# SmallEndian/antidote

Hardware: AMD Instinct MI355X
Metric: CRDT ops materialized/sec (whole node) + % HBM peak (higher is better)
Workload: dtype u64; 1 GPU; c3: antidote_crdt_set_aw, 1048576 keys x 1024 ops per GPU, D=8, 64-element universe; keys_per_gpu=1048576, ops_per_gpu=1073741824, n_dc=8, partitions=64, parallelism=partition-sharded x1, key_placement=rank r holds the keys with am_key_partition(key, 64) % N == r, step=GST min all-reduce (RCCL) + materialize all keys, base=fresh, zone_index=none

## Files before the change

### antidote_amd/csrc/am_group_split.h

```cpp
#pragma once

namespace amk_grp {

constexpr uint32_t IWB = 32;
__device__ __forceinline__ uint32_t wave_min_u32_v(uint32_t v) {
#define S_(C) v = min(v, dpp32<C>(v));
  AMK_ROW_STEPS(S_)
#undef S_
  v = min(v, (uint32_t)__shfl_xor((int)v, 16, WAVE));
  return min(v, (uint32_t)__shfl_xor((int)v, 32, WAVE));
}
struct ISlot {
  uint64_t off0, K, idb, key;
  uint32_t r, nops;
};
constexpr int SEGT = 4;
constexpr uint32_t SEGOPS = SEGT * 256;
template <int DMAX, bool LAG>
struct ISred {
  uint32_t mx[DMAX][WAVE];
};
template <int DMAX>
struct ISred<DMAX, true> {
  union {
    uint32_t mx[DMAX][WAVE];
    uint16_t list[SEGOPS];
  };
  uint32_t stage[SEGOPS / 32];
};
template <int DMAX, bool LAG>
struct ISmem : ISred<DMAX, LAG> {
  ISlot slot[IWB];
  uint64_t ct[DMAX][IWB];
  uint64_t mex[IWB];
  uint32_t count[IWB], pres[IWB];
  uint32_t flags[IWB];
};

template <int DMAX, int OPL, bool RANGE, class Ent>
__device__ __forceinline__ uint32_t incl_tile(const Ent &x, const PkRead<DMAX> &pk, uint64_t g, uint64_t off0,
                                              uint64_t off1, uint32_t (&mx)[DMAX], uint32_t &esc, uint32_t &cand) {
  uint32_t ib = 0;
#pragma unroll
  for (int k = 0; k < OPL; ++k) {
    const bool e = x.esc(k) == AM_PK_ESC;
    const bool inr = !RANGE || (g + k >= off0 && g + k < off1);
    bool in = inr && !e;
#pragma unroll
    for (int d = 0; d < DMAX; ++d) in = in && x(k, d) <= pk.thr[d];
    esc |= (uint32_t)(inr && e) << k;
    cand |= (uint32_t)(inr && !e) << k;
    if (in) {
#pragma unroll
      for (int d = 0; d < DMAX; ++d) mx[d] = max(mx[d], x(k, d));
    }
    ib |= (uint32_t)in << k;
  }
  return ib;
}

template <int DMAX>
__device__ __forceinline__ uint32_t mx_reduce(const uint32_t (*smx)[WAVE], uint32_t lane) {
  uint32_t m = 0;
  {
    const uint32_t d = lane >> 3, c = lane & 7u;
    if (d < (uint32_t)DMAX) {
      const u32x4 a0 = *(const u32x4 *)&smx[d][8 * c], a1 = *(const u32x4 *)&smx[d][8 * c + 4];
      m = max(max(max(a0.x, a0.y), max(a0.z, a0.w)), max(max(a1.x, a1.y), max(a1.z, a1.w)));
    }
    m = max(m, dpp32<0xB1>(m));
    m = max(m, dpp32<0x4E>(m));
    m = max(m, dpp32<0x141>(m));
  }
  uint32_t ql = lane;
  asm volatile("" : "+v"(ql));
  return (uint32_t)__builtin_amdgcn_ds_bpermute((int)((ql & 7u) << 5), (int)m);
}

#ifndef AM_INCL_WAVES
#define AM_INCL_WAVES(D) 4
#endif
#ifndef AM_INCL_LAG_WAVES
#define AM_INCL_LAG_WAVES(D) 5
#endif
template <int DMAX, int TYPE, bool EXACT, bool LAG>
__global__ void __launch_bounds__(BLOCK, LAG ? AM_INCL_LAG_WAVES(DMAX) : AM_INCL_WAVES(DMAX)) k_grp_incl(am_log_arg LA, am_read_batch B, am_read_result R, am_sel S,
                                                       am_retry next, am_retry routed, uint32_t short_opl,
                                                       uint32_t *ibm, uint64_t *escr) {
  const am_op_log L = LA.log();
  constexpr int OPL = 4;
  constexpr uint64_t TILE = (uint64_t)WAVE * OPL;
  constexpr uint32_t LPW = 32 / OPL;
  __shared__ ISmem<DMAX, LAG> smem[NW];
  ISmem<DMAX, LAG> &sm = smem[threadIdx.x >> 6];
  ISlot *sl = sm.slot;
  const uint32_t lane = threadIdx.x & (WAVE - 1);
  const uint32_t nd = EXACT ? (uint32_t)DMAX : L.n_dc;
  const uint64_t stride = L.snap_stride ? L.snap_stride : L.n_ops;
  const uint32_t sel0 = S.idx ? uniform_u32(S.range[0]) : 0u;
  const uint64_t nsel = S.idx ? (uint64_t)(uniform_u32(S.range[1]) - sel0) : B.n_reads;
  const uint64_t W = (uint64_t)gridDim.x * NW;
  const uint64_t gw = (uint64_t)blockIdx.x * NW + uniform_u32(threadIdx.x >> 6);
  const uint64_t n = B.n_reads;
  ReadU<DMAX> u;
  read_inputs<DMAX, false, true>(L, nd, B, 0, u);

  for (uint64_t b0 = gw * IWB; b0 < nsel; b0 += (uint64_t)IWB * W) {
    uint32_t sl_ = lane, sopl = short_opl;
    asm volatile("" : "+v"(sl_));
    asm volatile("" : "+s"(sopl));
    const uint64_t ii = b0 + sl_;
    bool elig = false, hand = false, route = false;
    uint64_t rr = 0;
    if (sl_ < IWB && ii < nsel) {
      GMeta mm;
      read_meta(L, B, S.idx ? (uint64_t)S.idx[sel0 + ii] : ii, TYPE, mm);
      rr = mm.r;
      if (mm.st != AM_OK) {
        R.status[mm.r] = mm.st, R.flags[mm.r] = 0;
      } else if (!wave_takes(L, B, mm, sopl)) {
        hand = true;
      } else if (LAG && routed.list && L.key_lag[mm.key * nd] == AM_LAG_ROUTED) {
        route = true;
      } else {
        elig = true;
        ISlot &w = sl[sl_];
        w.off0 = mm.off0, w.K = L.key_tbase[mm.key], w.idb = L.key_id_base ? L.key_id_base[mm.key] : 1;
        w.key = mm.key;
        w.r = (uint32_t)mm.r, w.nops = (uint32_t)(mm.off1 - mm.off0);
      }
    }
    const uint64_t hm = __ballot(hand);
    if (hm) {
      uint32_t base = 0;
      if (sl_ == 0) base = atomicAdd(next.count, (uint32_t)__popcll(hm));
      base = uniform_u32(base);
      if (hand) next.list[base + (uint32_t)__popcll(hm & ((1ull << sl_) - 1ull))] = (uint32_t)rr;
    }
    if (LAG) retry_append(routed, route, (uint32_t)rr, sl_);
    const uint64_t emask = __ballot(elig);
    uint32_t escmask = 0;
    uint64_t *const escw = escr + (gw * IWB) * WAVE;
    wave_sync();

    for (uint64_t em = emask; em; em &= em - 1) {
      const uint32_t j = (uint32_t)__builtin_ctzll(em);
      const uint64_t off0 = uniform_u64(sl[j].off0), off1 = off0 + uniform_u32(sl[j].nops);
      PkRead<DMAX> pk;
      pk_setup(u, nd, uniform_u64(sl[j].K), pk);
      uint32_t lb[DMAX];
      if (LAG) {
        const uint64_t key = uniform_u64(sl[j].key);
#pragma unroll
        for (int d = 0; d < DMAX; ++d) lb[d] = uniform_u32(d < (int)nd ? (uint32_t)L.key_lag[key * nd + d] : 0u);
      }
      uint32_t cnt = 0, minex = 0xFFFFFFFFu, anyc = 0, anyesc = 0;
      uint32_t mxr = 0;
      uint64_t escm = 0;
      const uint64_t t0 = off0 & ~31ull;
      if constexpr (LAG) {
        static_assert(OPL == 4 && TILE == 256 && SEGOPS == SEGT * TILE, "list entries: tile, lane, op of four");
        int64_t cinf = AM_IW_NOBOUND;
        int32_t lbm = INT32_MAX;
#pragma unroll
        for (int d = 0; d < DMAX; ++d)
          if (d < (int)nd) cinf = am_iw_fold(cinf, pk.thr[d], lb[d]), lbm = min(lbm, (int32_t)lb[d]);
        am_inclwin iw;
        am_iw_init(&iw, cinf, pk.never);
        const uint32_t cin_lim = am_iw_lim(iw.cin), out_lim = am_iw_lim(iw.hi);
        uint32_t in_lim = am_iw_in_lim(&iw);
        const uint32_t lo = (uint32_t)(off0 - t0), nops = (uint32_t)(off1 - off0);
        uint16_t *const list = sm.list;
        uint32_t *const stage = sm.stage;
        const uint32_t nt = (uint32_t)((off1 - 1 - t0) / TILE) + 1u;
        for (uint32_t sg = (nt + SEGT - 1) / SEGT; sg-- > 0;) {
          const uint64_t sb = t0 + (uint64_t)sg * SEGOPS;
          const uint32_t sr = sg * SEGOPS;
          uint32_t c[SEGT][OPL];
#pragma unroll
          for (int k = 0; k < SEGT; ++k) {
            const uint64_t g = sb + (uint64_t)k * TILE + (uint64_t)lane * OPL;
#pragma unroll
            for (int i = 0; i < OPL; ++i) c[k][i] = 0;
            if (g < off1) ld_n32<OPL>(L.lag_ct + g, c[k]);
          }
          if (in_lim < cin_lim) {
            uint32_t sure = 0;
#pragma unroll
            for (int k = 0; k < SEGT; ++k)
#pragma unroll
              for (int i = 0; i < OPL; ++i) {
                const uint32_t q = sr + (uint32_t)k * (uint32_t)TILE + lane * OPL + (uint32_t)i;
                if (q - lo < nops && c[k][i] < cin_lim) sure = max(sure, c[k][i] + 1u);
              }
            const uint32_t m = uniform_u32(wave_max_u32_v(sure));
            if (m) am_iw_raise(&iw, am_iw_cmax_sure(m - 1u)), in_lim = am_iw_in_lim(&iw);
          }
          uint32_t nl = 0;
          auto classify = [&](const int k, const uint32_t (&ck)[OPL]) {
            const uint64_t t = sb + (uint64_t)k * TILE;
            if (t >= off1) return;
            const uint32_t q = sr + (uint32_t)k * (uint32_t)TILE + lane * OPL;
            uint32_t *const sw = stage + k * (int)(TILE / 32) + lane / LPW;
            const bool whole = t >= off0 && t + TILE <= off1;
            if (whole) {
              const uint32_t ch = max(max(ck[0], ck[1]), max(ck[2], ck[3]));
              const uint32_t cl = min(min(ck[0], ck[1]), min(ck[2], ck[3]));
              const bool in = !__ballot(ch >= in_lim);
              if (in || !__ballot(cl < out_lim || ch == AM_PK_ESC)) {
                if (in) cnt += OPL;
                else minex = min(minex, q);
                anyc |= (1u << OPL) - 1u;
                if (lane % LPW == 0) *sw = in ? ~0u : 0u;
                return;
              }
            }
            uint32_t esc = 0, cand = 0, ib = 0, win = 0;
#pragma unroll
            for (int i = 0; i < OPL; ++i) {
              const bool inr = whole || q + (uint32_t)i - lo < nops;
              const int cl = am_iw_class32(ck[i], in_lim, out_lim);
              esc |= (uint32_t)(inr && cl == AM_IW_ESCAPED) << i;
              cand |= (uint32_t)(inr && cl != AM_IW_ESCAPED) << i;
              ib |= (uint32_t)(inr && cl == AM_IW_IN) << i;
              win |= (uint32_t)(inr && cl == AM_IW_WINDOW) << i;
            }
            cnt += (uint32_t)__popc(ib);
            anyc |= cand;
            anyesc |= esc;
            const uint32_t ti = q / (uint32_t)TILE;
            if (esc) escm |= ti < 64 / OPL ? (uint64_t)esc << (OPL * ti) : ~0ull;
            const uint32_t ex = cand & ~ib & ~win;
            if (ex) minex = min(minex, q + (uint32_t)__builtin_ctz(ex));
            uint32_t word = ib << (OPL * (lane % LPW));
#pragma unroll
            for (uint32_t xo = 1; xo < LPW; xo <<= 1) word |= (uint32_t)__shfl_xor((int)word, (int)xo);
            if (lane % LPW == 0) *sw = word;
            if (__ballot(win != 0)) {
              const uint32_t pc = (uint32_t)__popc(win);
              const uint32_t inc = wave_incl_scan_u32(pc, lane);
              const uint32_t tot = lane_u32(inc, WAVE - 1);
              uint32_t pos = nl + tot - inc;
#pragma unroll
              for (int i = OPL - 1; i >= 0; --i)
                if ((win >> i) & 1u) list[pos++] = (uint16_t)((uint32_t)k * (uint32_t)TILE + lane * OPL + (uint32_t)i);
              nl += tot;
            }
          };
#pragma unroll
          for (int k = SEGT - 1; k >= 0; --k) classify(k, c[k]);
          wave_sync();
          if (nl) {
            uint32_t mx[DMAX];
#pragma unroll
            for (int d = 0; d < DMAX; ++d) mx[d] = 0;
            const uint32_t *const cseg = L.lag_ct + sb;
            const uint16_t *const lseg = L.lag + sb;
            uint32_t cn = cseg[lane < nl ? (uint32_t)list[lane] : 0u];
            auto round = [&](const uint32_t r0, auto first) {
              const uint32_t i = r0 + lane;
              const bool v = i < nl;
              const uint32_t e = v ? (uint32_t)list[min(i, SEGOPS - 1u)] : 0u;
              const uint32_t cc = cn;
              uint32_t nx = 0;
              if (r0 + WAVE < nl) nx = cseg[i + WAVE < nl ? (uint32_t)list[min(i + WAVE, SEGOPS - 1u)] : 0u];
              bool need = v, sin = false;
              if constexpr (!decltype(first)::value) {
                const int cl = am_iw_class32(cc, in_lim, out_lim);
                sin = v && cl == AM_IW_IN, need = v && cl == AM_IW_WINDOW;
              }
              bool in = false;
              if (decltype(first)::value || __ballot(need)) {
                uint32_t lg[DMAX];
#pragma unroll
                for (int d = 0; d < DMAX; ++d) lg[d] = d < (int)nd ? (uint32_t)(lseg + (uint64_t)d * stride)[e] : 0u;
                in = need;
#pragma unroll
                for (int d = 0; d < DMAX; ++d) {
                  lg[d] = cc - (lb[d] + lg[d]);
                  in = in && lg[d] <= pk.thr[d];
                }
#pragma unroll
                for (int d = 0; d < DMAX; ++d) mx[d] = max(mx[d], in ? lg[d] : 0u);
              }
              cn = nx;
              const bool inc = in || sin;
              if (inc) atomicOr(stage + (e >> 5), 1u << (e & 31u));
              cnt += (uint32_t)inc;
              if (v && !inc) minex = min(minex, sr + e);
              if (__ballot(in)) {
                uint32_t f = 0xFFFFFFFFu;
#pragma unroll
                for (int d = 0; d < DMAX; ++d)
                  if (d < (int)nd) f = am_iw_fold32(f, mx[d], lb[d], lbm);
                am_iw_raise(&iw, am_iw_cmax_of32(uniform_u32(wave_max_u32_v(f)), lbm));
                in_lim = am_iw_in_lim(&iw);
              }
            };
            round(0u, std::true_type{});
            for (uint32_t r0 = WAVE; r0 < nl; r0 += WAVE) round(r0, std::false_type{});
            wave_sync();
#pragma unroll
            for (int d = 0; d < DMAX; ++d) sm.mx[d][lane] = mx[d];
          }
          {
            uint32_t wl = lane;
            asm volatile("" : "+v"(wl));
            const uint64_t w0 = sb + 32ull * wl;
            if (wl < SEGOPS / 32 && w0 < off1) {
              const uint32_t word = stage[wl];
              if (w0 >= off0 && w0 + 32 <= off1) {
                ibm[w0 >> 5] = word;
              } else {
                const uint32_t blo = off0 > w0 ? (uint32_t)(off0 - w0) : 0u;
                const uint32_t bhi = off1 < w0 + 32 ? (uint32_t)(off1 - w0) : 32u;
                const uint32_t mask = (bhi >= 32 ? ~0u : ((1u << bhi) - 1u)) & ~((1u << blo) - 1u);
                atomicAnd(ibm + (w0 >> 5), ~mask);
                atomicOr(ibm + (w0 >> 5), word & mask);
              }
            }
          }
          wave_sync();
          if (nl) mxr = max(mxr, mx_reduce<DMAX>(sm.mx, lane));
          wave_sync();
        }
      } else {
        uint32_t mx[DMAX];
#pragma unroll
        for (int d = 0; d < DMAX; ++d) mx[d] = 0;
        auto tile_out = [&](uint64_t t, uint64_t g, uint32_t ib, uint32_t esc, uint32_t cand) {
          if (pk.never) ib = 0;
          cnt += (uint32_t)__popc(ib);
          anyc |= cand;
          anyesc |= esc;
          const uint64_t ti = (t - t0) / TILE;
          if (esc) escm |= ti < 64 / OPL ? (uint64_t)esc << (OPL * ti) : ~0ull;
          const uint32_t ex = cand & ~ib;
          if (ex) minex = min(minex, (uint32_t)(g - t0) + (uint32_t)__builtin_ctz(ex));
          uint32_t word = ib << (OPL * (lane % LPW));
  #pragma unroll
          for (uint32_t xo = 1; xo < LPW; xo <<= 1) word |= (uint32_t)__shfl_xor((int)word, (int)xo);
          const uint64_t w0 = g & ~31ull;
          if (lane % LPW == 0 && w0 < off1) {
            if (w0 >= off0 && w0 + 32 <= off1) {
              ibm[w0 >> 5] = word;
            } else {
              const uint32_t lo = off0 > w0 ? (uint32_t)(off0 - w0) : 0u;
              const uint32_t hi = off1 < w0 + 32 ? (uint32_t)(off1 - w0) : 32u;
              const uint32_t mask = (hi >= 32 ? ~0u : ((1u << hi) - 1u)) & ~((1u << lo) - 1u);
              atomicAnd(ibm + (w0 >> 5), ~mask);
              atomicOr(ibm + (w0 >> 5), word & mask);
            }
          }
        };
        for (uint64_t t = t0; t < off1; t += TILE) {
          const uint64_t g = t + (uint64_t)lane * OPL;
          uint32_t esc = 0, cand = 0;
          const bool whole = t >= off0 && t + TILE <= off1;
          uint32_t x[OPL][DMAX];
#pragma unroll
          for (int d = 0; d < DMAX; ++d) {
            uint32_t q[OPL] = {};
            if (d < (int)nd && g < off1) ld_n32<OPL>(L.pk_vc + (uint64_t)d * stride + g, q);
#pragma unroll
            for (int k = 0; k < OPL; ++k) x[k][d] = q[k];
          }
          const uint32_t ib = whole ? incl_tile<DMAX, OPL, false>(pk_ent(x), pk, g, off0, off1, mx, esc, cand)
                                    : incl_tile<DMAX, OPL, true>(pk_ent(x), pk, g, off0, off1, mx, esc, cand);
          tile_out(t, g, ib, esc, cand);
        }
#pragma unroll
        for (int d = 0; d < DMAX; ++d) sm.mx[d][lane] = mx[d];
      }
      const uint32_t count_p = wave_sum_u32_v(cnt);
      minex = wave_min_u32_v(minex);
      const bool cands = __ballot(anyc != 0) != 0;
      const bool escs = __ballot(anyesc != 0) != 0;
      uint32_t mxd = mxr;
      if constexpr (!LAG) {
        wave_sync();
        mxd = mx_reduce<DMAX>(sm.mx, lane);
      }
      if (lane < nd) sm.ct[lane][j] = count_p ? pk.K + mxd : 0;
      if (lane == 0) {
        sm.flags[j] = cands ? pk.miss : 0u;
        sm.count[j] = count_p;
        sm.pres[j] = count_p ? u.allmask : 0u;
        sm.mex[j] = minex == 0xFFFFFFFFu ? NONE : t0 + minex;
      }
      if (escs) {
        escw[(uint64_t)j * WAVE + lane] = escm;
        escmask |= 1u << j;
      }
      wave_sync();
    }
    if (escmask) __builtin_amdgcn_s_waitcnt(0);
    for (uint32_t xm = escmask; xm; xm &= xm - 1) {
      const uint32_t j = (uint32_t)__builtin_ctz(xm);
      const uint64_t off0 = uniform_u64(sl[j].off0), off1 = off0 + uniform_u32(sl[j].nops);
      const uint64_t K = uniform_u64(sl[j].K), t0 = off0 & ~31ull;
      const uint64_t escm = escw[(uint64_t)j * WAVE + lane];
      Acc<DMAX> a;
      a.reset();
      const bool walk = __ballot(escm == ~0ull) != 0;
      const uint32_t *const escv = LAG ? L.lag_ct : L.pk_vc;
      for (uint64_t cur = walk ? off0 + lane : escm;;) {
        uint64_t p;
        if (walk) {
          while (cur < off1 && escv[cur] != AM_PK_ESC) cur += WAVE;
          if (cur >= off1) break;
          p = cur, cur += WAVE;
        } else {
          if (!cur) break;
          const uint32_t b = (uint32_t)__builtin_ctzll(cur);
          cur &= cur - 1;
          p = t0 + (uint64_t)(b / OPL) * TILE + (uint64_t)lane * OPL + b % OPL;
        }
        uint64_t sv[DMAX], ct;
        uint32_t meta;
        esc_load<DMAX>(L, nd, stride, p, LAG ? K : NONE, sv, ct, meta);
        if (eval_op<DMAX, false>(u, meta, ct, sv, u.allmask, false, p, a) && !(meta & AM_META_BAD))
          atomicOr(&ibm[p >> 5], 1u << (p & 31));
      }
      const uint32_t ecount = wave_sum_u32_v(a.count), eflags = wave_or_u32_v(a.flags);
      const uint32_t epres = wave_or_u32_v(a.pres);
      const uint64_t emex = wave_min_u64_v(a.min_excl);
      uint64_t emx = 0;
#pragma unroll
      for (int d = 0; d < DMAX; ++d) {
        if (d >= (int)nd) continue;
        const uint64_t am = wave_max_u64_v(a.mx[d]);
        if ((uint32_t)d == lane) emx = am;
      }
      if (lane < nd) sm.ct[lane][j] = umax64(sm.ct[lane][j], emx);
      if (lane == 0) {
        sm.flags[j] |= eflags;
        sm.count[j] += ecount;
        sm.pres[j] |= epres;
        sm.mex[j] = umin64(sm.mex[j], emex);
      }
    }
    wave_sync();
    uint32_t ol = lane;
    asm volatile("" : "+v"(ol));
    if (ol < IWB && (((uint32_t)emask >> ol) & 1u)) {
      const uint64_t r = sl[ol].r;
      const uint32_t flags = sm.flags[ol];
      const int32_t st = (flags & FLAG_BAD) ? AM_ERR_UNEXPECTED_OPERATION : AM_OK;
      R.status[r] = st;
      R.flags[r] = (uint8_t)(flags & 0xFFu);
      if (st == AM_OK) {
        const uint32_t c = sm.count[ol];
        const uint32_t opres = c == 0 ? 0u : sm.pres[ol];
        const uint64_t off0 = sl[ol].off0;
        R.new_last_op[r] = new_last_op_b(L, sl[ol].idb, off0, off0 + sl[ol].nops, sm.mex[ol]);
        R.last_ct_ignore[r] = c == 0 ? 1 : 0;
        R.last_ct_pres[r] = opres;
        R.is_new_ss[r] = c > 0;
        R.count[r] = c;
#pragma unroll
        for (int d = 0; d < DMAX; ++d)
          if (d < (int)nd) R.last_ct[(uint64_t)d * n + r] = ((opres >> d) & 1u) ? sm.ct[d][ol] : 0;
      }
    }
    wave_sync();
  }
}

constexpr uint32_t RLIST = 256;
struct RSlot {
  uint64_t off0, rk0, ooff;
  uint32_t r, nops, nrec, G, ocap, nb;
};
struct RSmem {
  uint32_t born[VG / 32], killed[VG / 32];
  uint32_t incl[VWORDS];
  uint16_t list[RLIST];
  uint16_t bri[VG];
  RSlot slot[IWB];
};
__device__ __forceinline__ void rec_apply(uint32_t x, uint32_t i, uint32_t sh, const uint32_t *incl, uint32_t *born,
                                          uint32_t *killed, uint16_t *bri) {
  if (x == 0xFFFFFFFFu) return;
  const uint32_t bit = AM_REC_OP(x) + sh;
  if (!((incl[bit >> 5] >> (bit & 31)) & 1u)) return;
  const uint32_t g = AM_REC_GRP(x);
  atomicOr(((x & AM_REC_KILL) ? killed : born) + (g >> 5), 1u << (g & 31));
  if (!(x & AM_REC_KILL)) bri[g] = (uint16_t)i;
}

template <int TYPE, bool SPANS, class Pre, class FPre, class FApply, class FAlive>
__device__ __forceinline__ void rec_pass(const am_op_log &L, const am_read_batch &B, am_read_result &R, const am_sel &S,
                                         uint32_t short_opl, const uint32_t *ibm, RSmem &s, uint32_t lane, FPre pre,
                                         FApply apply, FAlive alive) {
  const uint32_t sel0 = S.idx ? uniform_u32(S.range[0]) : 0u;
  const uint64_t nsel = S.idx ? (uint64_t)(uniform_u32(S.range[1]) - sel0) : B.n_reads;
  const uint64_t W = (uint64_t)gridDim.x * NW;
  const uint64_t gw = (uint64_t)blockIdx.x * NW + uniform_u32(threadIdx.x >> 6);
  const uint64_t *const pairs = L.prec ? L.prec : L.grp;
  auto prefetch = [&](uint32_t j, Pre &p) {
    const uint64_t off0 = s.slot[j].off0, t0 = off0 & ~31ull;
    const uint32_t nw = (uint32_t)((off0 + s.slot[j].nops - t0 + 31) / 32);
    p.w = lane < nw ? ibm[(t0 >> 5) + lane] : 0u;
    pre(j, p);
  };

  for (uint64_t b0 = gw * IWB; b0 < nsel; b0 += (uint64_t)IWB * W) {
    const uint64_t ii = b0 + lane;
    bool ok = false;
    if (lane < IWB && ii < nsel) {
      GMeta mm;
      read_meta(L, B, S.idx ? (uint64_t)S.idx[sel0 + ii] : ii, TYPE, mm);
      ok = mm.st == AM_OK && wave_takes(L, B, mm, short_opl) && R.status[mm.r] == AM_OK;
      if (ok) {
        RSlot &w = s.slot[lane];
        const uint64_t o0 = R.value.set_off[mm.r], o1 = R.value.set_off[mm.r + 1];
        w.off0 = mm.off0, w.rk0 = mm.rk0, w.ooff = o0;
        w.r = (uint32_t)mm.r, w.nops = (uint32_t)(mm.off1 - mm.off0), w.nrec = (uint32_t)(mm.rk1 - mm.rk0);
        if (SPANS) {
          const uint32_t nb = L.key_nspan[mm.key];
          w.nb = nb > w.nrec ? AM_NSPAN_NONE : nb;
        }
        w.G = mm.G, w.ocap = o1 - o0 < 0xFFFFFFFFull ? (uint32_t)(o1 - o0) : 0xFFFFFFFFu;
      }
    }
    uint64_t em = __ballot(ok);
    wave_sync();
    Pre cur;
    if (em) prefetch((uint32_t)__builtin_ctzll(em), cur);
    uint32_t setlen = 0;
    int32_t cap_err = 0;
    for (; em; em &= em - 1) {
      const uint32_t j = (uint32_t)__builtin_ctzll(em);
      const uint64_t off0 = uniform_u64(s.slot[j].off0), rk0 = uniform_u64(s.slot[j].rk0);
      const uint64_t off1 = off0 + uniform_u32(s.slot[j].nops);
      const uint32_t G = uniform_u32(s.slot[j].G);
      const uint64_t t0 = off0 & ~31ull;
      const uint32_t sh = (uint32_t)(off0 - t0), nw = (uint32_t)((off1 - t0 + 31) / 32);
      if (lane < nw) s.incl[lane] = cur.w;
      for (uint32_t i = WAVE + lane; i < nw; i += WAVE) s.incl[i] = ibm[(t0 >> 5) + i];
      for (uint32_t g = lane; g < (G + 31) / 32; g += WAVE) s.born[g] = 0, s.killed[g] = 0;
      const Pre now = cur;
      const uint64_t rest = em & (em - 1);
      if (rest) prefetch((uint32_t)__builtin_ctzll(rest), cur);
      wave_sync();
      apply(now, j, rk0, G, sh);
      wave_sync();
      const uint32_t aw = lane < (G + 31) / 32 ? alive(lane) : 0u;
      const uint32_t cnt = (uint32_t)__popc(aw);
      uint32_t ql = lane;
      asm volatile("" : "+v"(ql));
      const uint32_t inc = wave_incl_scan_u32(cnt, ql);
      const uint32_t ns = (uint32_t)__shfl((int)inc, 63, WAVE);
      const uint64_t ooff = uniform_u64(s.slot[j].ooff);
      const uint32_t ocap = uniform_u32(s.slot[j].ocap);
      const uint32_t nput = ns < ocap ? ns : ocap;
      for (uint32_t base = 0; base < nput; base += RLIST) {
        uint32_t o = inc - cnt;
        for (uint32_t bits = aw; bits; bits &= bits - 1, ++o)
          if (o >= base && o < base + RLIST) s.list[o - base] = (uint16_t)(lane * 32 + __builtin_ctz(bits));
        wave_sync();
        const uint32_t end = nput - base < RLIST ? nput - base : RLIST;
        for (uint32_t j0 = 0; j0 < end; j0 += 2 * WAVE) {
          const uint32_t j1 = j0 + lane, j2 = j1 + WAVE;
          u64x2 p1 = {0, 0}, p2 = {0, 0};
          if (j1 < end) p1 = *(const u64x2 *)(pairs + 2 * (rk0 + (L.prec ? s.bri[s.list[j1]] : s.list[j1])));
          if (j2 < end) p2 = *(const u64x2 *)(pairs + 2 * (rk0 + (L.prec ? s.bri[s.list[j2]] : s.list[j2])));
          if (j1 < end) R.value.set_a[ooff + base + j1] = p1.x, R.value.set_b[ooff + base + j1] = p1.y;
          if (j2 < end) R.value.set_a[ooff + base + j2] = p2.x, R.value.set_b[ooff + base + j2] = p2.y;
        }
        wave_sync();
      }
      if (lane == j) setlen = ns, cap_err = ns > ocap;
      wave_sync();
    }
    if (ok) {
      const uint64_t r = s.slot[lane].r;
      if (cap_err) R.status[r] = AM_ERR_CAPACITY;
      else R.value.set_len[r] = setlen;
    }
    wave_sync();
  }
}

constexpr uint32_t RCH = 512;
struct RPre {
  uint32_t w;
  u32x4 c[4];
};

template <int DMAX, int TYPE>
__global__ void __launch_bounds__(BLOCK, 5) k_grp_recs(am_log_arg LA, am_read_batch B, am_read_result R, am_sel S,
                                                       uint32_t short_opl, const uint32_t *ibm) {
  const am_op_log L = LA.log();
  __shared__ RSmem smem[NW];
  RSmem &s = smem[threadIdx.x >> 6];
  const uint32_t lane = threadIdx.x & (WAVE - 1);

  auto ld_recs = [&](uint64_t q0, uint64_t rk1, u32x4 (&c)[4]) {
#pragma unroll
    for (int k = 0; k < 4; ++k) {
      const uint64_t q = q0 + (uint64_t)k * 4 * WAVE + 4 * lane;
      c[k] = q < rk1 ? *(const u32x4 *)(L.rec_g + q) : u32x4{~0u, ~0u, ~0u, ~0u};
    }
  };
  auto pre = [&](uint32_t j, RPre &p) {
    const uint64_t rk0 = s.slot[j].rk0;
    ld_recs(rk0 & ~3ull, rk0 + s.slot[j].nrec, p.c);
  };
  auto apply4 = [&](const u32x4 (&c)[4], uint64_t q0, uint64_t rk0, uint64_t rk1, uint32_t sh) {
#pragma unroll
    for (int k = 0; k < 4; ++k) {
      const uint64_t q = q0 + (uint64_t)k * 4 * WAVE + 4 * lane;
      const uint32_t xs[4] = {c[k].x, c[k].y, c[k].z, c[k].w};
#pragma unroll
      for (int e = 0; e < 4; ++e) {
        if (xs[e] == 0xFFFFFFFFu || q + e < rk0 || q + e >= rk1) continue;
        rec_apply(xs[e], (uint32_t)(q + e - rk0), sh, s.incl, s.born, s.killed, s.bri);
      }
    }
  };
  auto apply = [&](const RPre &p, uint32_t j, uint64_t rk0, uint32_t, uint32_t sh) {
    const uint64_t rk1 = rk0 + uniform_u32(s.slot[j].nrec), qa = rk0 & ~3ull;
    apply4(p.c, qa, rk0, rk1, sh);
    for (uint64_t q0 = qa + 2 * RCH; q0 < rk1; q0 += 2 * RCH) {
      u32x4 c[4];
      ld_recs(q0, rk1, c);
      apply4(c, q0, rk0, rk1, sh);
    }
  };
  rec_pass<TYPE, false, RPre>(L, B, R, S, short_opl, ibm, s, lane, pre, apply,
                              [&](uint32_t w) { return s.born[w] & ~s.killed[w]; });
}

constexpr int SPRE = 4;
struct SPre {
  uint32_t w;
  u32x4 c[SPRE];
};

template <int DMAX, int TYPE>
__global__ void __launch_bounds__(BLOCK, 5) k_grp_spans(am_op_log L, am_read_batch B, am_read_result R, am_sel S,
                                                        uint32_t short_opl, const uint32_t *ibm) {
  __shared__ RSmem smem[NW];
  RSmem &s = smem[threadIdx.x >> 6];
  const uint32_t lane = threadIdx.x & (WAVE - 1);
  constexpr uint32_t SCH = (uint32_t)SPRE * 4 * WAVE;

  auto ld_spans = [&](uint64_t q0, uint64_t rk1, u32x4 (&c)[SPRE]) {
#pragma unroll
    for (int k = 0; k < SPRE; ++k) {
      const uint64_t q = q0 + (uint64_t)k * 4 * WAVE + 4 * lane;
      c[k] = q < rk1 ? *(const u32x4 *)(L.gspan + q) : u32x4{0, 0, 0, 0};
    }
  };
  auto pre = [&](uint32_t j, SPre &p) {
    const uint64_t rk0 = s.slot[j].rk0;
    const uint32_t nb = s.slot[j].nb;
    ld_spans(rk0 & ~3ull, rk0 + (nb == AM_NSPAN_NONE ? 0u : nb), p.c);
  };
  auto apply1 = [&](const u32x4 (&c)[SPRE], uint64_t q0, uint64_t rk0, uint64_t rk1, uint32_t sh) {
    uint32_t src[SPRE * 4];
    uint32_t am = 0;
#pragma unroll
    for (int k = 0; k < SPRE; ++k) {
      const uint64_t q = q0 + (uint64_t)k * 4 * WAVE + 4 * lane;
      const uint32_t xs[4] = {c[k].x, c[k].y, c[k].z, c[k].w};
#pragma unroll
      for (int e = 0; e < 4; ++e) {
        const bool inr = q + e >= rk0 && q + e < rk1;
        const uint32_t x = inr ? xs[e] : 0u;
        const uint32_t b = (x & 0xFFFFu) + sh, kl = (x >> 16) + sh;
        const bool inb = (s.incl[b >> 5] >> (b & 31)) & 1u, ink = (s.incl[kl >> 5] >> (kl & 31)) & 1u;
        const bool al = inr && inb && (kl == b || !ink);
        src[4 * k + e] = al ? L.gsrc[q + e] : 0u;
        am |= (uint32_t)al << (4 * k + e);
      }
    }
#pragma unroll
    for (int i = 0; i < SPRE * 4; ++i)
      if ((am >> i) & 1u) {
        const uint32_t g = src[i] & 0xFFFFu;
        atomicOr(s.born + (g >> 5), 1u << (g & 31));
        s.bri[g] = (uint16_t)(src[i] >> 16);
      }
  };
  auto apply = [&](const SPre &p, uint32_t j, uint64_t rk0, uint32_t G, uint32_t sh) {
    const uint32_t nbj = uniform_u32(s.slot[j].nb);
    const bool byrec = nbj == AM_NSPAN_NONE;
    const uint64_t rk1 = rk0 + (byrec ? 0u : nbj), qa = rk0 & ~3ull;
    apply1(p.c, qa, rk0, rk1, sh);
    for (uint64_t q0 = qa + SCH; q0 < rk1; q0 += SCH) {
      u32x4 c[SPRE];
      ld_spans(q0, rk1, c);
      apply1(c, q0, rk0, rk1, sh);
    }
    if (byrec) {
      const uint32_t nrec = uniform_u32(s.slot[j].nrec);
      for (uint32_t i = lane; i < nrec; i += WAVE) rec_apply(L.rec_g[rk0 + i], i, sh, s.incl, s.born, s.killed, s.bri);
      wave_sync();
      for (uint32_t g = lane; g < (G + 31) / 32; g += WAVE) s.born[g] &= ~s.killed[g];
    }
  };
  rec_pass<TYPE, true, SPre>(L, B, R, S, short_opl, ibm, s, lane, pre, apply, [&](uint32_t w) { return s.born[w]; });
}

template <int D, int TYPE, bool EXACT>
int launch_split(am_ctx *ctx, const am_op_log *L, const am_read_batch *B, am_read_result *R, am_sel S,
                 am_retry next, uint32_t short_opl) {
  const uint64_t stride = L->snap_stride ? L->snap_stride : L->n_ops;
  void *ibm = nullptr;
  if (int rc = am_ctx_scratch(ctx, AM_SCR_INCL, (stride / 32 + 4) * 4, &ibm)) return rc;
  const bool lag = L->lag_ct && L->lag && L->key_lag;
  const bool spans = L->key_nspan && L->gspan && L->gsrc;
  static int occ_i[2] = {0, 0}, occ_w = 0, occ_s = 0;
  const uint64_t want = (B->n_reads + NW * IWB - 1) / (NW * IWB);
  const uint64_t bp = grp_grid(ctx, occ_i[0], k_grp_incl<D, TYPE, EXACT, false>, BLOCK, 0, 2, want);
  const uint64_t bi = lag ? grp_grid(ctx, occ_i[1], k_grp_incl<D, TYPE, EXACT, true>, BLOCK, 0, 2, want) : bp;
  const uint64_t bw = spans ? grp_grid(ctx, occ_s, k_grp_spans<D, TYPE>, BLOCK, 0, 1, want)
                            : grp_grid(ctx, occ_w, k_grp_recs<D, TYPE>, BLOCK, 0, 1, want);
  if (bi == 0) return AM_OK;
  void *escv = nullptr;
  if (int rc = am_ctx_scratch(ctx, AM_SCR_ESCM, (bi > bp ? bi : bp) * NW * IWB * WAVE * sizeof(uint64_t), &escv))
    return rc;
  uint64_t *const escr = (uint64_t *)escv;
  if (lag) {
    am_retry routed;
    am_sel rsel;
    if (int rc = am_route_list(ctx, B->n_reads, &routed, &rsel)) return rc;
    hipLaunchKernelGGL((k_grp_incl<D, TYPE, EXACT, true>), dim3((unsigned)bi), dim3(BLOCK), 0, ctx->stream, *L, *B, *R,
                       S, next, routed, short_opl, (uint32_t *)ibm, escr);
    hipLaunchKernelGGL((k_grp_incl<D, TYPE, EXACT, false>), dim3((unsigned)bp), dim3(BLOCK), 0, ctx->stream, *L, *B,
                       *R, rsel, next, am_retry{}, short_opl, (uint32_t *)ibm, escr);
  } else {
    hipLaunchKernelGGL((k_grp_incl<D, TYPE, EXACT, false>), dim3((unsigned)bp), dim3(BLOCK), 0, ctx->stream, *L, *B,
                       *R, S, next, am_retry{}, short_opl, (uint32_t *)ibm, escr);
  }
  if (spans) {
    hipLaunchKernelGGL((k_grp_spans<D, TYPE>), dim3((unsigned)bw), dim3(BLOCK), 0, ctx->stream, *L, *B, *R, S,
                       short_opl, (const uint32_t *)ibm);
  } else {
    hipLaunchKernelGGL((k_grp_recs<D, TYPE>), dim3((unsigned)bw), dim3(BLOCK), 0, ctx->stream, *L, *B, *R, S,
                       short_opl, (const uint32_t *)ibm);
  }
  AM_HIP(hipGetLastError());
  return AM_OK;
}

}
```

### antidote_amd/csrc/am_inclwin.h

```cpp
#pragma once
#include <stdint.h>

#if defined(__HIPCC__)
#define AM_IW_HD __host__ __device__ __forceinline__
#else
#define AM_IW_HD static inline
#endif

#define AM_IW_LAG_MAX 0xFFFFll
#define AM_IW_ESC 0xFFFFFFFFu

enum { AM_IW_ESCAPED = 0, AM_IW_OUT = 1, AM_IW_IN = 2, AM_IW_WINDOW = 3 };

typedef struct am_inclwin {
  int64_t cin;
  int64_t hi;
  int64_t cmax;
} am_inclwin;

#define AM_IW_NOBOUND INT64_MAX
AM_IW_HD int64_t am_iw_fold(int64_t acc, uint32_t v, uint32_t lb) {
  const int64_t t = (int64_t)v + (int64_t)(int32_t)lb;
  return t < acc ? t : acc;
}
AM_IW_HD void am_iw_init(am_inclwin *w, int64_t cin_fold, int never) {
  const int64_t cin = (never || cin_fold == AM_IW_NOBOUND) ? -1 - AM_IW_LAG_MAX : cin_fold;
  w->cin = cin, w->hi = cin + AM_IW_LAG_MAX, w->cmax = -1;
}
AM_IW_HD void am_iw_setup(am_inclwin *w, const uint32_t *thr, const uint32_t *lb, uint32_t nd, int never) {
  int64_t f = AM_IW_NOBOUND;
  for (uint32_t d = 0; d < nd; ++d) f = am_iw_fold(f, thr[d], lb[d]);
  am_iw_init(w, f, never);
}

AM_IW_HD int64_t am_iw_cmax_of(const uint32_t *m, const uint32_t *lb, uint32_t nd) {
  int64_t f = AM_IW_NOBOUND;
  for (uint32_t d = 0; d < nd; ++d) f = am_iw_fold(f, m[d], lb[d]);
  return nd ? f : -1;
}
AM_IW_HD int64_t am_iw_cmax_sure(uint32_t c) { return (int64_t)c - AM_IW_LAG_MAX; }
AM_IW_HD void am_iw_raise(am_inclwin *w, int64_t cmax) { w->cmax = cmax > w->cmax ? cmax : w->cmax; }

AM_IW_HD uint32_t am_iw_fold32(uint32_t acc, uint32_t m, uint32_t lb, int32_t lbm) {
#if defined(__HIPCC__)
  const uint32_t t = __builtin_elementwise_add_sat(m, lb - (uint32_t)lbm);
#else
  const uint32_t s = m + (lb - (uint32_t)lbm), t = s < m ? 0xFFFFFFFFu : s;
#endif
  return t < acc ? t : acc;
}
AM_IW_HD int64_t am_iw_cmax_of32(uint32_t f, int32_t lbm) { return (int64_t)f + (int64_t)lbm; }

AM_IW_HD int am_iw_sure_in(const am_inclwin *w, uint32_t c) { return c != AM_IW_ESC && (int64_t)c <= w->cin; }
AM_IW_HD int am_iw_class(const am_inclwin *w, uint32_t c) {
  if (c == AM_IW_ESC) return AM_IW_ESCAPED;
  if ((int64_t)c > w->hi) return AM_IW_OUT;
  if ((int64_t)c <= (w->cin < w->cmax ? w->cin : w->cmax)) return AM_IW_IN;
  return AM_IW_WINDOW;
}

AM_IW_HD uint32_t am_iw_lim(int64_t v) { return v < 0 ? 0u : v >= 0xFFFFFFFEll ? 0xFFFFFFFFu : (uint32_t)v + 1u; }
AM_IW_HD uint32_t am_iw_in_lim(const am_inclwin *w) { return am_iw_lim(w->cin < w->cmax ? w->cin : w->cmax); }
AM_IW_HD int am_iw_class32(uint32_t c, uint32_t in_lim, uint32_t out_lim) {
  if (c == AM_IW_ESC) return AM_IW_ESCAPED;
  if (c >= out_lim) return AM_IW_OUT;
  return c < in_lim ? AM_IW_IN : AM_IW_WINDOW;
}
```

Baseline: 305.8 billion ops/s.

## Precompute per-slot thresholds and window limits in LDS slots, shrink ct to u32

Moves the per-key threshold, lag bounds and inclusion-window limit setup from the wave-serial per-slot loop into the parallel slot-fill phase, storing the results in an enlarged per-slot LDS struct. The window raise logic is rewritten to work directly on 32-bit limits instead of 64-bit state. It also stores ct as a u32 delta and adds K back at output time. Escape-path maxima now go through a global scratch buffer, and the read inputs are re-read on every batch iteration. The gains are less serial per-key work and smaller LDS footprint, at the cost of larger slot structs, extra global scratch traffic and redundant input reads.

```diff
diff --git a/antidote_amd/csrc/am_group_split.h b/antidote_amd/csrc/am_group_split.h
--- a/antidote_amd/csrc/am_group_split.h
+++ b/antidote_amd/csrc/am_group_split.h
@@ -10,9 +10,21 @@
   v = min(v, (uint32_t)__shfl_xor((int)v, 16, WAVE));
   return min(v, (uint32_t)__shfl_xor((int)v, 32, WAVE));
 }
-struct ISlot {
-  uint64_t off0, K, idb, key;
+constexpr uint32_t SLOT_NEVER = 1u, SLOT_MISS = 2u;
+struct ISlotHead {
+  uint64_t off0, K, idb;
   uint32_t r, nops;
+};
+template <int DMAX, bool LAG>
+struct alignas(16) ISlot : ISlotHead {
+  uint32_t thr[DMAX];
+  uint32_t fl;
+};
+template <int DMAX>
+struct alignas(16) ISlot<DMAX, true> : ISlotHead {
+  uint32_t thr[DMAX];
+  uint32_t lb[DMAX];
+  uint32_t lbm, cin_lim, out_lim, fl;
 };
 constexpr int SEGT = 4;
 constexpr uint32_t SEGOPS = SEGT * 256;
@@ -30,12 +42,13 @@
 };
 template <int DMAX, bool LAG>
 struct ISmem : ISred<DMAX, LAG> {
-  ISlot slot[IWB];
-  uint64_t ct[DMAX][IWB];
+  ISlot<DMAX, LAG> slot[IWB];
+  uint32_t ct[DMAX][IWB];
   uint64_t mex[IWB];
   uint32_t count[IWB], pres[IWB];
   uint32_t flags[IWB];
 };
+constexpr uint32_t FLAG_INVIEW = 0x200u;
 
 template <int DMAX, int OPL, bool RANGE, class Ent>
 __device__ __forceinline__ uint32_t incl_tile(const Ent &x, const PkRead<DMAX> &pk, uint64_t g, uint64_t off0,
@@ -93,7 +106,7 @@
   constexpr uint32_t LPW = 32 / OPL;
   __shared__ ISmem<DMAX, LAG> smem[NW];
   ISmem<DMAX, LAG> &sm = smem[threadIdx.x >> 6];
-  ISlot *sl = sm.slot;
+  ISlot<DMAX, LAG> *sl = sm.slot;
   const uint32_t lane = threadIdx.x & (WAVE - 1);
   const uint32_t nd = EXACT ? (uint32_t)DMAX : L.n_dc;
   const uint64_t stride = L.snap_stride ? L.snap_stride : L.n_ops;
@@ -102,8 +115,7 @@
   const uint64_t W = (uint64_t)gridDim.x * NW;
   const uint64_t gw = (uint64_t)blockIdx.x * NW + uniform_u32(threadIdx.x >> 6);
   const uint64_t n = B.n_reads;
-  ReadU<DMAX> u;
-  read_inputs<DMAX, false, true>(L, nd, B, 0, u);
+  const uint32_t allmask = nd >= 32 ? 0xFFFFFFFFu : ((1u << nd) - 1u);
 
   for (uint64_t b0 = gw * IWB; b0 < nsel; b0 += (uint64_t)IWB * W) {
     uint32_t sl_ = lane, sopl = short_opl;
@@ -112,6 +124,8 @@
     const uint64_t ii = b0 + sl_;
     bool elig = false, hand = false, route = false;
     uint64_t rr = 0;
+    ReadU<DMAX> u;
+    read_inputs<DMAX, false, true>(L, nd, B, 0, u);
     if (sl_ < IWB && ii < nsel) {
       GMeta mm;
       read_meta(L, B, S.idx ? (uint64_t)S.idx[sel0 + ii] : ii, TYPE, mm);
@@ -124,10 +138,25 @@
         route = true;
       } else {
         elig = true;
-        ISlot &w = sl[sl_];
-        w.off0 = mm.off0, w.K = L.key_tbase[mm.key], w.idb = L.key_id_base ? L.key_id_base[mm.key] : 1;
-        w.key = mm.key;
+        const uint64_t K = L.key_tbase[mm.key];
+        uint32_t lbk[DMAX], thr[DMAX];
+        if (LAG) {
+#pragma unroll
+          for (int d = 0; d < DMAX; ++d) lbk[d] = d < (int)nd ? (uint32_t)L.key_lag[mm.key * nd + d] : 0u;
+        }
+        am_iw_read rs;
+        am_iw_read_setup(u.S, u.spres, u.allmask, K, LAG ? lbk : nullptr, nd, (uint32_t)DMAX, thr, &rs);
+        ISlot<DMAX, LAG> &w = sl[sl_];
+        w.off0 = mm.off0, w.K = K, w.idb = L.key_id_base ? L.key_id_base[mm.key] : 1;
         w.r = (uint32_t)mm.r, w.nops = (uint32_t)(mm.off1 - mm.off0);
+#pragma unroll
+        for (int d = 0; d < DMAX; ++d) w.thr[d] = thr[d];
+        w.fl = (rs.never ? SLOT_NEVER : 0u) | (rs.miss ? SLOT_MISS : 0u);
+        if constexpr (LAG) {
+#pragma unroll
+          for (int d = 0; d < DMAX; ++d) w.lb[d] = lbk[d];
+          w.lbm = (uint32_t)rs.lbm, w.cin_lim = rs.cin_lim, w.out_lim = rs.out_lim;
+        }
       }
     }
     const uint64_t hm = __ballot(hand);
@@ -147,12 +176,14 @@
       const uint32_t j = (uint32_t)__builtin_ctzll(em);
       const uint64_t off0 = uniform_u64(sl[j].off0), off1 = off0 + uniform_u32(sl[j].nops);
       PkRead<DMAX> pk;
-      pk_setup(u, nd, uniform_u64(sl[j].K), pk);
+#pragma unroll
+      for (int d = 0; d < DMAX; ++d) pk.thr[d] = uniform_u32(sl[j].thr[d]);
+      const uint32_t sfl = uniform_u32(sl[j].fl);
+      pk.never = (sfl & SLOT_NEVER) != 0;
       uint32_t lb[DMAX];
-      if (LAG) {
-        const uint64_t key = uniform_u64(sl[j].key);
-#pragma unroll
-        for (int d = 0; d < DMAX; ++d) lb[d] = uniform_u32(d < (int)nd ? (uint32_t)L.key_lag[key * nd + d] : 0u);
+      if constexpr (LAG) {
+#pragma unroll
+        for (int d = 0; d < DMAX; ++d) lb[d] = uniform_u32(sl[j].lb[d]);
       }
       uint32_t cnt = 0, minex = 0xFFFFFFFFu, anyc = 0, anyesc = 0;
       uint32_t mxr = 0;
@@ -160,15 +191,9 @@
       const uint64_t t0 = off0 & ~31ull;
       if constexpr (LAG) {
         static_assert(OPL == 4 && TILE == 256 && SEGOPS == SEGT * TILE, "list entries: tile, lane, op of four");
-        int64_t cinf = AM_IW_NOBOUND;
-        int32_t lbm = INT32_MAX;
-#pragma unroll
-        for (int d = 0; d < DMAX; ++d)
-          if (d < (int)nd) cinf = am_iw_fold(cinf, pk.thr[d], lb[d]), lbm = min(lbm, (int32_t)lb[d]);
-        am_inclwin iw;
-        am_iw_init(&iw, cinf, pk.never);
-        const uint32_t cin_lim = am_iw_lim(iw.cin), out_lim = am_iw_lim(iw.hi);
-        uint32_t in_lim = am_iw_in_lim(&iw);
+        const int32_t lbm = (int32_t)uniform_u32(sl[j].lbm);
+        const uint32_t cin_lim = uniform_u32(sl[j].cin_lim), out_lim = uniform_u32(sl[j].out_lim);
+        uint32_t in_lim = 0;
         const uint32_t lo = (uint32_t)(off0 - t0), nops = (uint32_t)(off1 - off0);
         uint16_t *const list = sm.list;
         uint32_t *const stage = sm.stage;
@@ -194,7 +219,7 @@
                 if (q - lo < nops && c[k][i] < cin_lim) sure = max(sure, c[k][i] + 1u);
               }
             const uint32_t m = uniform_u32(wave_max_u32_v(sure));
-            if (m) am_iw_raise(&iw, am_iw_cmax_sure(m - 1u)), in_lim = am_iw_in_lim(&iw);
+            if (m) in_lim = min(cin_lim, am_iw_lim_raise(in_lim, am_iw_lim_sure(m - 1u)));
           }
           uint32_t nl = 0;
           auto classify = [&](const int k, const uint32_t (&ck)[OPL]) {
@@ -293,8 +318,7 @@
 #pragma unroll
                 for (int d = 0; d < DMAX; ++d)
                   if (d < (int)nd) f = am_iw_fold32(f, mx[d], lb[d], lbm);
-                am_iw_raise(&iw, am_iw_cmax_of32(uniform_u32(wave_max_u32_v(f)), lbm));
-                in_lim = am_iw_in_lim(&iw);
+                in_lim = min(cin_lim, am_iw_lim_raise(in_lim, am_iw_lim_of32(uniform_u32(wave_max_u32_v(f)), lbm)));
               }
             };
             round(0u, std::true_type{});
@@ -381,11 +405,13 @@
         wave_sync();
         mxd = mx_reduce<DMAX>(sm.mx, lane);
       }
-      if (lane < nd) sm.ct[lane][j] = count_p ? pk.K + mxd : 0;
+      uint32_t cl_ = lane;
+      asm volatile("" : "+v"(cl_));
+      if (cl_ < nd) sm.ct[cl_][j] = mxd;
       if (lane == 0) {
-        sm.flags[j] = cands ? pk.miss : 0u;
+        sm.flags[j] = ((cands && (sfl & SLOT_MISS)) ? (uint32_t)AM_FLAG_MISSING_DC_LOGGED : 0u) | (count_p ? FLAG_INVIEW : 0u);
         sm.count[j] = count_p;
-        sm.pres[j] = count_p ? u.allmask : 0u;
+        sm.pres[j] = count_p ? allmask : 0u;
         sm.mex[j] = minex == 0xFFFFFFFFu ? NONE : t0 + minex;
       }
       if (escs) {
@@ -394,7 +420,10 @@
       }
       wave_sync();
     }
-    if (escmask) __builtin_amdgcn_s_waitcnt(0);
+    if (escmask) {
+      __builtin_amdgcn_s_waitcnt(0);
+      read_inputs<DMAX, false, true>(L, nd, B, 0, u);
+    }
     for (uint32_t xm = escmask; xm; xm &= xm - 1) {
       const uint32_t j = (uint32_t)__builtin_ctz(xm);
       const uint64_t off0 = uniform_u64(sl[j].off0), off1 = off0 + uniform_u32(sl[j].nops);
@@ -432,7 +461,7 @@
         const uint64_t am = wave_max_u64_v(a.mx[d]);
         if ((uint32_t)d == lane) emx = am;
       }
-      if (lane < nd) sm.ct[lane][j] = umax64(sm.ct[lane][j], emx);
+      if (lane < nd) escw[(uint64_t)j * WAVE + lane] = emx;
       if (lane == 0) {
         sm.flags[j] |= eflags;
         sm.count[j] += ecount;
@@ -440,6 +469,7 @@
         sm.mex[j] = umin64(sm.mex[j], emex);
       }
     }
+    if (escmask) __builtin_amdgcn_s_waitcnt(0);
     wave_sync();
     uint32_t ol = lane;
     asm volatile("" : "+v"(ol));
@@ -458,9 +488,15 @@
         R.last_ct_pres[r] = opres;
         R.is_new_ss[r] = c > 0;
         R.count[r] = c;
+        const uint64_t K = sl[ol].K;
+        const bool inview = (flags & FLAG_INVIEW) != 0, esc = ((escmask >> ol) & 1u) != 0;
 #pragma unroll
         for (int d = 0; d < DMAX; ++d)
-          if (d < (int)nd) R.last_ct[(uint64_t)d * n + r] = ((opres >> d) & 1u) ? sm.ct[d][ol] : 0;
+          if (d < (int)nd) {
+            uint64_t v = inview ? K + sm.ct[d][ol] : 0;
+            if (esc) v = umax64(v, escw[(uint64_t)ol * WAVE + d]);
+            R.last_ct[(uint64_t)d * n + r] = ((opres >> d) & 1u) ? v : 0;
+          }
       }
     }
     wave_sync();
diff --git a/antidote_amd/csrc/am_inclwin.h b/antidote_amd/csrc/am_inclwin.h
--- a/antidote_amd/csrc/am_inclwin.h
+++ b/antidote_amd/csrc/am_inclwin.h
@@ -66,3 +66,55 @@
   if (c >= out_lim) return AM_IW_OUT;
   return c < in_lim ? AM_IW_IN : AM_IW_WINDOW;
 }
+AM_IW_HD uint32_t am_iw_lim_sure(uint32_t c) { return c > 0xFFFEu ? c - 0xFFFEu : 0u; }
+AM_IW_HD uint32_t am_iw_lim_of32(uint32_t f, int32_t lbm) {
+  if (lbm >= 0) {
+    const uint32_t s = f + (uint32_t)lbm;
+    return (s < f || s >= 0xFFFFFFFEu) ? 0xFFFFFFFFu : s + 1u;
+  }
+  const uint32_t n = 0u - (uint32_t)lbm;
+  return f < n ? 0u : f - n + 1u;
+}
+AM_IW_HD uint32_t am_iw_lim_raise(uint32_t cmax_lim, uint32_t lim) { return lim > cmax_lim ? lim : cmax_lim; }
+
+typedef struct am_iw_read {
+  int never;
+  int miss;
+  int32_t lbm;
+  uint32_t cin_lim;
+  uint32_t out_lim;
+} am_iw_read;
+#if defined(__HIPCC__)
+#define AM_IW_UNROLL _Pragma("unroll")
+#else
+#define AM_IW_UNROLL
+#endif
+AM_IW_HD uint32_t am_iw_thr(uint64_t s, uint64_t K) {
+  return s < K ? 0u : (s - K >= (uint64_t)AM_IW_ESC ? AM_IW_ESC - 1u : (uint32_t)(s - K));
+}
+AM_IW_HD void am_iw_read_setup(const uint64_t *S, uint32_t spres, uint32_t allmask, uint64_t K, const uint32_t *lb,
+                               uint32_t nd, uint32_t dmax, uint32_t *thr, am_iw_read *o) {
+  int64_t f = 0;
+  int32_t lbm = INT32_MAX;
+  const int miss = (allmask & ~spres) != 0;
+  int never = miss;
+  AM_IW_UNROLL
+  for (uint32_t d = 0; d < dmax; ++d) {
+    if (d >= nd) {
+      thr[d] = AM_IW_ESC;
+      continue;
+    }
+    const uint64_t s = ((spres >> d) & 1u) ? S[d] : 0u;
+    never |= s < K;
+    thr[d] = am_iw_thr(s, K);
+    if (lb) {
+      const int64_t t = (int64_t)thr[d] + (int64_t)(int32_t)lb[d];
+      f = (d == 0 || t < f) ? t : f;
+      lbm = (int32_t)lb[d] < lbm ? (int32_t)lb[d] : lbm;
+    }
+  }
+  am_inclwin w;
+  am_iw_init(&w, (lb && nd) ? f : AM_IW_NOBOUND, never);
+  o->never = never, o->miss = miss, o->lbm = lbm;
+  o->cin_lim = am_iw_lim(w.cin), o->out_lim = am_iw_lim(w.hi);
+}
```

Result: faster. 322.9 billion ops/s (median of 6 runs) (+5.6%).
